# Julian-Wyatt/AnoDDPM

Measured on AMD Instinct MI355X. Metric: reverse-diffusion images/sec @256x256 T=1000 simplex, higher is better.
Workload: dtype f32; 1 GPU; 256x256 simplex(8 oct) T=1000 base128 attn16,8 batch4/GPU (BASELINE config 2); per_gpu_batch=4, global_batch=4, T=1000, parallelism=batch-sharded x1 (no data-path collective), output_finite=True

## Files before the change

anoddpm_amd/csrc/attention.hip:

```cpp
#include "common.h"

namespace {

typedef float f32x4 __attribute__((ext_vector_type(4)));

constexpr int AT_LMAX = 1024;
constexpr int AT_WAVES = 8;
constexpr int AT_NT = AT_WAVES * 64;

template <int CHQ>
__global__ __launch_bounds__(AT_NT) void attention_kernel(const anoddpm_attention_args a)
{
    constexpr int CH = CHQ * 16;
    constexpr int QP = CH + 4;
    constexpr int TPW = CHQ >= AT_WAVES ? CHQ / AT_WAVES : 1;
    __shared__ __attribute__((aligned(16))) float lds[16 * (AT_LMAX + 4) + 16 * QP];
    const int L = a.L, SP = L + 4;
    float *S = lds, *Qs = lds + 16 * (AT_LMAX + 4);
    const int tid = threadIdx.x, lane = tid & 63, wave = tid >> 6;
    const int l16 = lane & 15, kq = lane >> 4;
    const int row0 = blockIdx.x * 16, hd = blockIdx.y, b = blockIdx.z;
    const int C3 = 3 * a.heads * CH;
    const float *__restrict__ qkv = a.qkv + (int64_t)b * L * C3 + hd * 3 * CH;
    const int nkt = L >> 4;

    for (int idx = tid; idx < 16 * (CH / 4); idx += AT_NT) {
        const int r = idx / (CH / 4), c4 = idx - r * (CH / 4);
        *reinterpret_cast<f32x4 *>(Qs + r * QP + c4 * 4) = *reinterpret_cast<const f32x4 *>(qkv + (int64_t)(row0 + r) * C3 + c4 * 4);
    }
    constexpr bool DB = CHQ < 32;
    f32x4 kb[DB ? 2 : 1][CHQ];
    auto load_k = [&](f32x4 (&dst)[CHQ], int jt) {
        const float *kp = qkv + (int64_t)(jt * 16 + l16) * C3 + CH + kq * 4;
#pragma unroll
        for (int g = 0; g < CHQ; ++g) dst[g] = *reinterpret_cast<const f32x4 *>(kp + g * 16);
    };
    constexpr int NACC = CHQ >= 32 ? 4 : 1;
    auto score_tile = [&](const f32x4 (&kk)[CHQ], int jt) {
        f32x4 acc[NACC];
#pragma unroll
        for (int c = 0; c < NACC; ++c) acc[c] = f32x4{0.f, 0.f, 0.f, 0.f};
#pragma unroll
        for (int g = 0; g < CHQ; ++g) {
            const f32x4 qa = *reinterpret_cast<const f32x4 *>(Qs + l16 * QP + g * 16 + kq * 4);
#pragma unroll
            for (int e = 0; e < 4; ++e) acc[g % NACC] = __builtin_amdgcn_mfma_f32_16x16x4f32(qa[e], kk[g][e], acc[g % NACC], 0, 0, 0);
        }
        if constexpr (NACC == 4) acc[0] = (acc[0] + acc[1]) + (acc[2] + acc[3]);
#pragma unroll
        for (int r = 0; r < 4; ++r) S[(kq * 4 + r) * SP + jt * 16 + l16] = acc[0][r] * a.scale;
    };
    if (wave < nkt) load_k(kb[0], wave);
    __syncthreads();
    if constexpr (DB) {
        for (int jt = wave; jt < nkt; jt += 2 * AT_WAVES) {
            if (jt + AT_WAVES < nkt) load_k(kb[1], jt + AT_WAVES);
            score_tile(kb[0], jt);
            if (jt + AT_WAVES < nkt) {
                if (jt + 2 * AT_WAVES < nkt) load_k(kb[0], jt + 2 * AT_WAVES);
                score_tile(kb[1], jt + AT_WAVES);
            }
        }
    } else {
        for (int jt = wave; jt < nkt; jt += AT_WAVES) {
            if (jt != wave) load_k(kb[0], jt);
            score_tile(kb[0], jt);
        }
    }
    const int ct0 = wave * TPW;
    const bool pv_active = ct0 < CHQ;
    float vb[2][TPW][4];
    auto load_v = [&](float (&dst)[TPW][4], int kg) {
        const float *vp = qkv + (int64_t)(kg * 16 + kq * 4) * C3 + 2 * CH + ct0 * 16 + l16;
#pragma unroll
        for (int t = 0; t < TPW; ++t)
#pragma unroll
            for (int e = 0; e < 4; ++e) dst[t][e] = vp[(int64_t)e * C3 + t * 16];
    };
    if (pv_active) load_v(vb[0], 0);
    __syncthreads();

    {
        constexpr int TPR = AT_NT / 16;
        const int r = tid / TPR, sub = tid % TPR;
        float *srow = S + r * SP;
        float m = -INFINITY;
        for (int j = sub; j < L; j += TPR) m = fmaxf(m, srow[j]);
#pragma unroll
        for (int o = TPR / 2; o >= 1; o >>= 1) m = fmaxf(m, __shfl_xor(m, o, TPR));
        float sum = 0.f;
        for (int j = sub; j < L; j += TPR) {
            const float e = __expf(srow[j] - m);
            srow[j] = e;
            sum += e;
        }
#pragma unroll
        for (int o = TPR / 2; o >= 1; o >>= 1) sum += __shfl_xor(sum, o, TPR);
        const float inv = 1.0f / sum;
        float *prow = a.probs ? a.probs + (((int64_t)b * a.heads + hd) * L + row0 + r) * L : nullptr;
        for (int j = sub; j < L; j += TPR) {
            const float p = srow[j] * inv;
            srow[j] = p;
            if (prow) prow[j] = p;
        }
    }
    __syncthreads();

    if (!pv_active) return;
    f32x4 oacc[TPW];
#pragma unroll
    for (int t = 0; t < TPW; ++t) oacc[t] = f32x4{0.f, 0.f, 0.f, 0.f};
    auto pv_group = [&](const float (&vv)[TPW][4], int kg) {
        const f32x4 pa = *reinterpret_cast<const f32x4 *>(S + l16 * SP + kg * 16 + kq * 4);
#pragma unroll
        for (int e = 0; e < 4; ++e)
#pragma unroll
            for (int t = 0; t < TPW; ++t) oacc[t] = __builtin_amdgcn_mfma_f32_16x16x4f32(pa[e], vv[t][e], oacc[t], 0, 0, 0);
    };
    for (int kg = 0; kg < nkt; kg += 2) {
        if (kg + 1 < nkt) load_v(vb[1], kg + 1);
        pv_group(vb[0], kg);
        if (kg + 1 < nkt) {
            if (kg + 2 < nkt) load_v(vb[0], kg + 2);
            pv_group(vb[1], kg + 1);
        }
    }
    float *__restrict__ O = a.out + ((int64_t)b * L + row0 + kq * 4) * (a.heads * CH) + hd * CH + ct0 * 16 + l16;
#pragma unroll
    for (int t = 0; t < TPW; ++t)
#pragma unroll
        for (int r = 0; r < 4; ++r) O[(int64_t)r * (a.heads * CH) + t * 16] = oacc[t][r];
}

}

extern "C" int anoddpm_attention(const anoddpm_attention_args *a, void *stream)
{
    ANODDPM_REQUIRE(a && a->qkv && a->out, "attention: null pointer");
    ANODDPM_REQUIRE(a->B >= 1 && a->heads >= 1 && a->B <= 65535 && a->heads <= 65535, "attention: bad batch / head count");
    ANODDPM_REQUIRE(a->L >= 16 && a->L % 16 == 0 && a->L <= AT_LMAX, "attention: L must be a multiple of 16 in [16, 1024]");
    ANODDPM_REQUIRE(a->ch >= 16 && a->ch <= 512 && (a->ch & (a->ch - 1)) == 0, "attention: head width must be a power of two in [16, 512]");
    ANODDPM_REQUIRE(((uintptr_t)a->qkv & 15) == 0, "attention: qkv must be 16-byte aligned");
    const dim3 grid((unsigned)(a->L / 16), (unsigned)a->heads, (unsigned)a->B);
    hipStream_t s = anoddpm::as_stream(stream);
    switch (a->ch / 16) {
        case 1: hipLaunchKernelGGL((attention_kernel<1>), grid, dim3(AT_NT), 0, s, *a); break;
        case 2: hipLaunchKernelGGL((attention_kernel<2>), grid, dim3(AT_NT), 0, s, *a); break;
        case 4: hipLaunchKernelGGL((attention_kernel<4>), grid, dim3(AT_NT), 0, s, *a); break;
        case 8: hipLaunchKernelGGL((attention_kernel<8>), grid, dim3(AT_NT), 0, s, *a); break;
        case 16: hipLaunchKernelGGL((attention_kernel<16>), grid, dim3(AT_NT), 0, s, *a); break;
        default: hipLaunchKernelGGL((attention_kernel<32>), grid, dim3(AT_NT), 0, s, *a); break;
    }
    return anoddpm::check_launch("attention");
}
```

anoddpm_amd/csrc/winograd.hip:

```cpp
#include "buf_load.h"
#include "common.h"

using anoddpm::buf_load4;
using anoddpm::buf_rsrc;
using anoddpm::f32x4;
using anoddpm::silu_f;

namespace {

typedef float f32x16 __attribute__((ext_vector_type(16)));

constexpr int WKC = 16;

constexpr int DPITCH = 5;

template <bool FAST, int WMW, int WNW, bool PROBE = false, bool VSH = false>
__global__ __launch_bounds__(128 * WMW * WNW, 2) void wino_kernel(const anoddpm_igemm_args a)
{
    unsigned long long tstamp[5];
    if (PROBE) tstamp[0] = __builtin_amdgcn_s_memtime();
    constexpr int NT = 128 * WMW * WNW;
    constexpr int WBN = 32 * WNW;
    constexpr int PROWS = 8 * WMW + 2;
    constexpr int WPATCH = PROWS * 18;
    constexpr int PJ = (WPATCH * 4 + NT - 1) / NT;
    constexpr int SLOTPX = PJ * NT / 4;
    constexpr int DT_F4 = SLOTPX * DPITCH;
    constexpr int EX_FLOATS = (WMW * WNW) * 2 * 8 * 4 * 64;
    constexpr int V_F4 = 16 * 4 * 32;
    constexpr int LDS_FLOATS = VSH ? (2 * DT_F4 + 2 * V_F4) * 4 : EX_FLOATS;
    __shared__ __attribute__((aligned(16))) float lds[LDS_FLOATS];
    static_assert(VSH ? (EX_FLOATS <= LDS_FLOATS && WNW == 4 && WMW == 1) : (2 * DT_F4 * 4 <= EX_FLOATS), "LDS layout");
    static_assert(PJ * NT >= WPATCH * 4 && PJ * NT <= SLOTPX * 4, "staging slots");
    f32x4 *ldsD = reinterpret_cast<f32x4 *>(lds);

    const int tid = threadIdx.x;
    const int lane = tid & 63, wave = tid >> 6;
    const int xh = __builtin_amdgcn_readfirstlane(wave / (WMW * WNW));
    const int wm = (wave / WNW) & (WMW - 1), wn = wave & (WNW - 1);
    const int h = lane >> 5, l31 = lane & 31;

    const int H = a.H, W = a.W;
    const int K = a.c0 + a.c1, N = a.N, K4 = K >> 2;
    const int bx = blockIdx.x % (W >> 4), by = blockIdx.x / (W >> 4);
    const int y0 = by * (8 * WMW), x0 = bx * 16;
    const int n0 = blockIdx.y * WBN;
    const int ksplit = a.ksplit;
    const int ksi = blockIdx.z % ksplit;
    const int b = blockIdx.z / ksplit;
    const int a_mode = a.a_mode;

    const float *A0 = a.a0 + (int64_t)b * a.a0_bs;
    const float *A1 = a.a1 ? a.a1 + (int64_t)b * a.a1_bs : nullptr;
    const float *gsc = a.gn_scale ? a.gn_scale + (int64_t)b * a.gn_ld : nullptr;
    const float *gsh = a.gn_shift ? a.gn_shift + (int64_t)b * a.gn_ld : nullptr;
    const bool affine = (gsc != nullptr);
    const bool act = a.act != 0;
    const int nchunks_all = K / WKC;
    const int cps = (nchunks_all + ksplit - 1) / ksplit;
    const int cbeg = ksi * cps;
    const int nchunks = cbeg + cps < nchunks_all ? cbeg + cps : nchunks_all;

    int spix[PJ];
    const int pq = tid & 3;
#pragma unroll
    for (int j = 0; j < PJ; ++j) {
        const int idx = tid + j * NT;
        const int p = idx >> 2;
        const int py = p / 18, px = p - py * 18;
        const int gy = y0 + py - 1, gx = x0 + px - 1;
        int sp = -1;
        if (p < WPATCH && gy >= 0 && gy < H && gx >= 0 && gx < W)
            sp = (a_mode == 0) ? gy * W + gx : (gy >> 1) * (W >> 1) + (gx >> 1);
        spix[j] = sp;
    }
    f32x4 praw[PJ];
    f32x4 asc = {1.f, 1.f, 1.f, 1.f}, ash = {0.f, 0.f, 0.f, 0.f};
    const __amdgpu_buffer_rsrc_t rA0 = buf_rsrc(A0), rA1 = buf_rsrc(A1 ? A1 : A0);
    const __amdgpu_buffer_rsrc_t rSc = buf_rsrc(gsc ? gsc : A0), rSh = buf_rsrc(gsh ? gsh : A0);
    auto load_patch = [&](int chunk) {
        const int kbase = chunk * WKC;
        const bool first = kbase < a.c0;
// ... 137 lines not shown
                __builtin_amdgcn_sched_barrier(0);
#pragma unroll
                for (int v = 0; v < 4; ++v)
#pragma unroll
                    for (int kk = 0; kk < 4; ++kk)
                        acc[uu * 4 + v] = __builtin_amdgcn_mfma_f32_32x32x2f32(af[set][v][kk], bvr[uu][v][kk], acc[uu * 4 + v], 0, 0, 0);
                __builtin_amdgcn_sched_barrier(0);
                if (g4 < 2) load_b(chunk, 1, uu, uu);
                else        load_b(nxt, 0, uu, uu);
                if (g4 == 0) store_patch(chunk & 1);
                if (g4 == 1) t_write((chunk + 1) & 1);
                if (g4 == 2) load_patch(nxt3);
            }
        }
    } else {
        load_patch(cbeg);
        store_patch(cbeg & 1);
        load_patch(cbeg < last ? cbeg + 1 : last);
        load_b(cbeg, 0, 0, 0);
        load_b(cbeg, 0, 1, 1);
        __syncthreads();
        issue_reads(cbeg & 1, 0, 0, 0);
        issue_reads(cbeg & 1, 0, 0, 1);
        make_av(0);
        if (PROBE) tstamp[1] = __builtin_amdgcn_s_memtime();
        for (int chunk = cbeg; chunk < nchunks; ++chunk) {
            const int nxt = chunk < last ? chunk + 1 : last;
            const int nxt2 = chunk + 2 < nchunks ? chunk + 2 : last;
    #pragma unroll
            for (int g4 = 0; g4 < 4; ++g4) {
                const int uu = g4 & 1;
                if (g4 == 3) __syncthreads();
                const int rbuf = g4 < 3 ? (chunk & 1) : ((chunk + 1) & 1);
                const int rkg = g4 < 3 ? (g4 + 1) >> 1 : 0, ruu = (g4 + 1) & 1;
                issue_reads(rbuf, rkg, ruu, 0);
                __builtin_amdgcn_sched_barrier(0);
    #pragma unroll
                for (int v = 0; v < 2; ++v)
    #pragma unroll
                    for (int kk = 0; kk < 4; ++kk)
                        acc[uu * 4 + v] = __builtin_amdgcn_mfma_f32_32x32x2f32(av[v][kk], bvr[uu][v][kk], acc[uu * 4 + v], 0, 0, 0);
                __builtin_amdgcn_sched_barrier(0);
                issue_reads(rbuf, rkg, ruu, 1);
                __builtin_amdgcn_sched_barrier(0);
    #pragma unroll
                for (int v = 2; v < 4; ++v)
    #pragma unroll
                    for (int kk = 0; kk < 4; ++kk)
                        acc[uu * 4 + v] = __builtin_amdgcn_mfma_f32_32x32x2f32(av[v][kk], bvr[uu][v][kk], acc[uu * 4 + v], 0, 0, 0);
                __builtin_amdgcn_sched_barrier(0);
                if (g4 < 2) load_b(chunk, 1, uu, uu);
                else        load_b(nxt, 0, uu, uu);
                if (g4 == 0) {
                    store_patch((chunk + 1) & 1);
                    load_patch(nxt2);
                }
                make_av(ruu);
            }
        }

    }
    if (PROBE) tstamp[2] = __builtin_amdgcn_s_memtime();
    auto partial = [&](int r, float (&out4)[4]) {
        float tm[2][4];
#pragma unroll
        for (int v = 0; v < 4; ++v) {
            const float m0 = acc[v][r], m1 = acc[4 + v][r];
            if (xh == 0) { tm[0][v] = m0 + m1; tm[1][v] = m1; }
            else         { tm[0][v] = m0;      tm[1][v] = -m0 - m1; }
        }
#pragma unroll
        for (int i = 0; i < 2; ++i) {
            out4[i * 2 + 0] = tm[i][0] + tm[i][1] + tm[i][2];
            out4[i * 2 + 1] = tm[i][1] - tm[i][2] - tm[i][3];
        }
    };
    const int n = n0 + bcol;
    const bool nok = n < N;
    const int nc = nok ? n : 0;
    const bool part = ksplit > 1;
    float *__restrict__ O = part ? a.ws + ((int64_t)ksi * a.B + b) * ((int64_t)H * W) * N : a.out + (int64_t)b * a.o_bs;
    const int o_ld = part ? N : a.out_ld;
    const float alpha = part ? 1.f : a.alpha;
    const float *__restrict__ R = (a.res && !part) ? a.res + (int64_t)b * a.r_bs : nullptr;
    float add = 0.f;
    if (a.bias && !part) add += a.bias[nc];
    if (a.temb && !part) add += a.temb[(int64_t)b * a.temb_ld + nc];
    float cs = 0.f, cq = 0.f;
    float rv[8][4];
#pragma unroll
    for (int rr = 0; rr < 8; ++rr) {
        const int r = xh * 8 + rr;
        const int row = (r & 3) + 8 * (r >> 2) + 4 * h;
        const int tile = wm * 32 + row;
        const int oy = y0 + 2 * (tile >> 3), ox = x0 + 2 * (tile & 7);
#pragma unroll
        for (int e = 0; e < 4; ++e)
            rv[rr][e] = R ? R[((int64_t)(oy + (e >> 1)) * W + ox + (e & 1)) * a.res_ld + nc] : 0.f;
    }
    float *ex = lds;
    const int pair = wave & (WMW * WNW - 1);
    if (xh == 0) {
#pragma unroll
        for (int rr = 0; rr < 8; ++rr) {
            float p4[4];
            partial(8 + rr, p4);
#pragma unroll
            for (int e = 0; e < 4; ++e) ex[(((pair * 2 + 0) * 8 + rr) * 4 + e) * 64 + lane] = p4[e];
        }
    } else {
#pragma unroll
        for (int rr = 0; rr < 8; ++rr) {
            float p4[4];
            partial(rr, p4);
#pragma unroll
            for (int e = 0; e < 4; ++e) ex[(((pair * 2 + 1) * 8 + rr) * 4 + e) * 64 + lane] = p4[e];
        }
    }
    __syncthreads();
    if (PROBE) tstamp[3] = __builtin_amdgcn_s_memtime();

    auto finalize = [&](int rbase) {
#pragma unroll
        for (int rr = 0; rr < 8; ++rr) {
            const int r = rbase + rr;
            const int row = (r & 3) + 8 * (r >> 2) + 4 * h;
            const int tile = wm * 32 + row;
            const int oy = y0 + 2 * (tile >> 3), ox = x0 + 2 * (tile & 7);
            float p4[4];
            partial(r, p4);
#pragma unroll
            for (int e = 0; e < 4; ++e) {
                const float other = ex[(((pair * 2 + (1 - xh)) * 8 + rr) * 4 + e) * 64 + lane];
                const float v = alpha * (p4[e] + other) + add + rv[rr][e];
                if (nok) {
                    O[((int64_t)(oy + (e >> 1)) * W + ox + (e & 1)) * o_ld + nc] = v;
                    cs += v;
                    cq += v * v;
                }
            }
        }
    };
    if (xh == 0) finalize(0); else finalize(8);
    if (a.stats && !part) {
        float *st = a.stats + ((int64_t)b * (gridDim.x * 2 * WMW) + blockIdx.x * (2 * WMW) + wm * 2 + xh) * N * 2;
        const float s2 = cs + __shfl_xor(cs, 32);
        const float q2 = cq + __shfl_xor(cq, 32);
        if (h == 0 && nok) { st[n * 2] = s2; st[n * 2 + 1] = q2; }
    }
    if (PROBE) {
        __builtin_amdgcn_s_waitcnt(0);
        tstamp[4] = __builtin_amdgcn_s_memtime();
        if (tid == 0) {
            unsigned long long *dbg = reinterpret_cast<unsigned long long *>(a.ws) +
                                      (size_t)(blockIdx.x + gridDim.x * (blockIdx.y + gridDim.y * blockIdx.z)) * 8;
            for (int i = 0; i < 5; ++i) dbg[i] = tstamp[i];
        }
    }
}

}

namespace anoddpm {

int launch_winograd(const anoddpm_igemm_args *a, hipStream_t s)
{
    ANODDPM_REQUIRE(a->ks == 3 && a->b_mode == 0 && a->heads == 1, "winograd: needs a 3x3 conv with packed weights");
    ANODDPM_REQUIRE(a->a_mode == 0 || a->a_mode == 1, "winograd: pooled operand loads use the direct kernel");
    ANODDPM_REQUIRE(a->H % 16 == 0 && a->W % 16 == 0, "winograd: H and W must be multiples of 16");
    const int K = a->c0 + a->c1;
    ANODDPM_REQUIRE(K % WKC == 0 && (a->c1 == 0 || a->c0 % WKC == 0), "winograd: channel counts must be multiples of 16");
    const int cps = (K / WKC + a->ksplit - 1) / a->ksplit;
    ANODDPM_REQUIRE((a->ksplit - 1) * cps < K / WKC, "winograd: ksplit leaves a block without channels");
    ANODDPM_REQUIRE(a->ksplit == 1 || !a->stats || a->stats_rows >= 1, "winograd: split-K statistics need stats_rows");
    const int dbg = anoddpm::g_debug[0];
    const int wmw = dbg == 1 ? 2 : 1;
    const bool fast = a->gn_scale && a->act;
#ifdef ANODDPM_ABLATE
    const bool probe = anoddpm::g_debug[1] == 1 && fast && a->ksplit == 1 && a->ws && wmw == 1;
#else
    const bool probe = false;
#endif
    const int wnw = (wmw == 1 && dbg != 2 && !probe && a->N % 128 == 0) ? 4 : 2;
    const int wbn = 32 * wnw;
    dim3 grid((unsigned)wino_tiles(a->H, a->W, wmw), (unsigned)((a->N + wbn - 1) / wbn), (unsigned)(a->B * a->ksplit));
    ANODDPM_REQUIRE(grid.y <= 65535 && (int64_t)a->B * a->ksplit <= 65535, "winograd: grid too large");
    ANODDPM_REQUIRE((int64_t)16 * K * a->N * 4 < ((int64_t)1 << 31), "winograd: transformed weights exceed 32-bit buffer offsets");
    ANODDPM_REQUIRE((int64_t)a->H * a->W * (a->a0_ld > a->a1_ld ? a->a0_ld : a->a1_ld) * 4 < ((int64_t)1 << 31),
                    "winograd: operand slice exceeds 32-bit buffer offsets");
    if (wmw == 2) {
        if (fast) hipLaunchKernelGGL((wino_kernel<true, 2, 2>), grid, dim3(512), 0, s, *a);
        else      hipLaunchKernelGGL((wino_kernel<false, 2, 2>), grid, dim3(512), 0, s, *a);
#ifdef ANODDPM_ABLATE
    } else if (probe) {
        hipLaunchKernelGGL((wino_kernel<true, 1, 2, true>), grid, dim3(256), 0, s, *a);
#endif
    } else if (wnw == 4 && dbg != 3) {
        if (fast) hipLaunchKernelGGL((wino_kernel<true, 1, 4, false, true>), grid, dim3(512), 0, s, *a);
        else      hipLaunchKernelGGL((wino_kernel<false, 1, 4, false, true>), grid, dim3(512), 0, s, *a);
    } else if (wnw == 4) {
        if (fast) hipLaunchKernelGGL((wino_kernel<true, 1, 4>), grid, dim3(512), 0, s, *a);
        else      hipLaunchKernelGGL((wino_kernel<false, 1, 4>), grid, dim3(512), 0, s, *a);
    } else {
        if (fast) hipLaunchKernelGGL((wino_kernel<true, 1, 2>), grid, dim3(256), 0, s, *a);
        else      hipLaunchKernelGGL((wino_kernel<false, 1, 2>), grid, dim3(256), 0, s, *a);
    }
    return check_launch("winograd");
}

}
```

anoddpm_amd/csrc/executor.hip:

```cpp
#include <stdarg.h>
#include <string.h>
#include <vector>
#include "common.h"

namespace anoddpm {

static thread_local char g_err[512] = "";
int g_debug[16] = {0};

void set_error(const char *fmt, ...)
{
    va_list ap;
    va_start(ap, fmt);
    vsnprintf(g_err, sizeof(g_err), fmt, ap);
    va_end(ap);
}

struct ProfState {
    bool on = false;
    std::vector<hipEvent_t> pool;
    std::vector<int> codes;
    std::vector<float> last_ms;
    std::vector<int> last_codes;
    size_t used = 0;
    double ms[ANODDPM_OP_MAX] = {0};
    int64_t launches[ANODDPM_OP_MAX] = {0};
};
static ProfState g_prof;

#define ANODDPM_OPS(X) \
    X(IGEMM,            anoddpm_igemm_args,            anoddpm_igemm) \
    X(GN_STATS,         anoddpm_gn_args,               anoddpm_gn_stats) \
    X(SOFTMAX,          anoddpm_softmax_args,          anoddpm_softmax_rows) \
    X(RESAMPLE,         anoddpm_resample_args,         anoddpm_resample2x) \
    X(LINEAR,           anoddpm_linear_args,           anoddpm_linear_small) \
    X(POSEMB,           anoddpm_posemb_args,           anoddpm_posemb) \
    X(STEM,             anoddpm_stem_args,             anoddpm_conv_stem) \
    X(LAYOUT,           anoddpm_layout_args,           anoddpm_nhwc_to_nchw) \
    X(CHAN_STATS,       anoddpm_chan_stats_args,       anoddpm_chan_stats) \
    X(HEAD,             anoddpm_head_args,             anoddpm_conv_head) \
    X(GN_FINALIZE,      anoddpm_gn_finalize_args,      anoddpm_gn_finalize) \
    X(WGRAD3,           anoddpm_wgrad_args,            anoddpm_conv3x3_wgrad) \
    X(WGRAD1,           anoddpm_wgrad1_args,           anoddpm_wgrad_pointwise) \
    X(GN_BWD,           anoddpm_gn_bwd_args,           anoddpm_gn_silu_backward) \
    X(PACK,             anoddpm_pack_args,             anoddpm_pack_weights) \
    X(SOFTMAX_BWD,      anoddpm_softmax_bwd_args,      anoddpm_softmax_rows_backward) \
    X(TRANSPOSE,        anoddpm_transpose_args,        anoddpm_transpose_square) \
    X(LINEAR_BWD,       anoddpm_linear_bwd_args,       anoddpm_linear_small_backward) \
    X(STEM_BWD,         anoddpm_stem_bwd_args,         anoddpm_conv_stem_backward) \
    X(HEAD_BWD,         anoddpm_head_bwd_args,         anoddpm_conv_head_backward) \
    X(COLSUM_FOLD,      anoddpm_colsum_fold_args,      anoddpm_colsum_fold) \
    X(ATTENTION,        anoddpm_attention_args,        anoddpm_attention) \
    X(PACK_BATCH,       anoddpm_pack_batch_args,       anoddpm_pack_batch) \
    X(DROPOUT,          anoddpm_dropout_args,          anoddpm_dropout) \
    X(LINEAR_BWD_BATCH, anoddpm_linear_bwd_batch_args, anoddpm_linear_small_backward_batch)

static int dispatch(const anoddpm_op &op, void *stream)
{
    switch (op.code) {
#define X(code, args_t, fn) case ANODDPM_OP_##code: return fn(static_cast<const args_t *>(op.args), stream);
        ANODDPM_OPS(X)
#undef X
        default: set_error("run_ops: unknown op code %d", op.code); return ANODDPM_EINVAL;
    }
}

}

using namespace anoddpm;

extern "C" int anoddpm_internal_variant(int32_t key, int32_t value)
{
    if (key < 0 || key >= 16) return ANODDPM_EINVAL;
#ifndef ANODDPM_ABLATE
    if (!(key == 0 || key == 4 || key == 5 || key == 8 || key == 9)) {
        set_error("internal_variant: key %d selects a timing ablation; this library was built without ANODDPM_ABLATE", key);
        return ANODDPM_EINVAL;
    }
#endif
    g_debug[key] = value;
    return ANODDPM_OK;
}

extern "C" int anoddpm_ablate_build(void)
{
#ifdef ANODDPM_ABLATE
    return 1;
#else
    return 0;
#endif
}

extern "C" int anoddpm_abi_version(void) { return ANODDPM_ABI_VERSION; }

extern "C" const char *anoddpm_last_error(void) { return g_err; }

extern "C" int anoddpm_device_count(void)
{
    int n = 0;
    if (hipGetDeviceCount(&n) != hipSuccess) { (void)hipGetLastError(); return 0; }
    return n;
}

extern "C" int anoddpm_run_ops(const anoddpm_op *ops, int32_t n, void *stream)
{
    ANODDPM_REQUIRE(ops || n == 0, "run_ops: null op list");
    for (int i = 0; i < n; ++i) {
        ANODDPM_REQUIRE(ops[i].args, "run_ops: op %d has null args", i);
        hipEvent_t e0 = nullptr, e1 = nullptr;
        const bool prof = g_prof.on && ops[i].code > 0 && ops[i].code < ANODDPM_OP_MAX;
        if (prof) {
            if (g_prof.used + 2 > g_prof.pool.size()) {
                hipEvent_t a, b;
                if (hipEventCreate(&a) != hipSuccess || hipEventCreate(&b) != hipSuccess) {
                    set_error("run_ops: hipEventCreate failed");
                    return ANODDPM_ELAUNCH;
                }
                g_prof.pool.push_back(a);
                g_prof.pool.push_back(b);
            }
            e0 = g_prof.pool[g_prof.used];
            e1 = g_prof.pool[g_prof.used + 1];
            g_prof.used += 2;
            const int icfg = ops[i].code == ANODDPM_OP_IGEMM ? static_cast<const anoddpm_igemm_args *>(ops[i].args)->cfg : 0;
            const bool w43 = ops[i].code == ANODDPM_OP_WGRAD3 && static_cast<const anoddpm_wgrad_args *>(ops[i].args)->algo == 1;
            g_prof.codes.push_back((icfg == 2 || icfg == 6) ? 12 : ((icfg == 3 || icfg == 7) ? 14 : (icfg == 5 ? 13 : (w43 ? 15 : ops[i].code))));
            (void)hipEventRecord(e0, as_stream(stream));
        }
        const int rc = dispatch(ops[i], stream);
        if (prof) (void)hipEventRecord(e1, as_stream(stream));
        if (rc != ANODDPM_OK) {
            char tmp[400];
            strncpy(tmp, g_err, sizeof(tmp) - 1);
            tmp[sizeof(tmp) - 1] = 0;
            set_error("op %d (code %d): %s", i, ops[i].code, tmp);
            return rc;
        }
    }
    return ANODDPM_OK;
}

extern "C" int anoddpm_prof_enable(int32_t enable)
{
    g_prof.on = enable != 0;
    if (enable) {
        g_prof.used = 0;
        g_prof.codes.clear();
        memset(g_prof.ms, 0, sizeof(g_prof.ms));
        memset(g_prof.launches, 0, sizeof(g_prof.launches));
    }
    return ANODDPM_OK;
}

extern "C" int anoddpm_prof_active(void) { return g_prof.on ? 1 : 0; }

extern "C" int anoddpm_prof_collect(double *ms_per_code, int64_t *launches_per_code)
{
    ANODDPM_REQUIRE(ms_per_code && launches_per_code, "prof_collect: null pointer");
// ... 50 lines not shown
```

anoddpm_amd/csrc/smallmap.hip:

```cpp
#include "buf_load.h"
#include "common.h"
#include "gn_stats.h"

using anoddpm::buf_load4;
using anoddpm::buf_rsrc;
using anoddpm::f32x4;
using anoddpm::silu_f;
using anoddpm::uniform;

namespace {

constexpr int SM_NT = 512;

__host__ __device__ constexpr int sm_kch(int ks) { return ks == 3 ? 256 : 512; }
__host__ __device__ constexpr int sm_hpix(int ks, int tm, int w) { return ks == 1 ? tm : (tm / w + 2) * (w + 2); }

template <int KS, int RT, int CT, int LOG2W>
__global__ __launch_bounds__(SM_NT) void smallmap_kernel(const anoddpm_igemm_args a)
{
    constexpr int TM = 16 * RT, TN = 16 * CT, TAPS = KS * KS;
    constexpr int KCH = sm_kch(KS), PITCH = KCH + 4;
    constexpr int CPW = KCH / 8;
    constexpr int SPT = CPW / 16;
    constexpr int SPC = TAPS * SPT;
    constexpr int PD = KS == 3 ? 6 : 4;
    constexpr int W = 1 << LOG2W;
    constexpr int HPIX = sm_hpix(KS, TM, W);
    constexpr int HP = W + 2;
    constexpr int QPP = KCH / 4;
    constexpr int PPI = SM_NT / QPP;
    constexpr int NI = (HPIX + PPI - 1) / PPI;
    constexpr int RP = TN + 4;
    static_assert(SPC % PD == 0, "ring slots must be static");
    extern __shared__ __attribute__((aligned(16))) float lds[];

    const int tid = threadIdx.x, lane = tid & 63;
    const int wave = __builtin_amdgcn_readfirstlane(tid >> 6);
    const int l16 = lane & 15, q = lane >> 4;
    const int K = a.c0 + a.c1, K4 = K >> 2, N = a.N;
    const int P = a.H * a.W;
    const int nchunks = (K + KCH - 1) / KCH;
    const int Kpad = nchunks * KCH;
    const int nbuf = nchunks > 1 ? 2 : 1;
    float *aff_sc = lds, *aff_sh = lds + Kpad;
    float *Abuf = lds + 2 * Kpad;
    float *red = Abuf;

    const int n0 = blockIdx.x * TN;
    const int p0g = blockIdx.y * TM;
    const int b = p0g / P, p0 = p0g - b * P;
    const int y0 = p0 >> LOG2W;
    const float *A0 = a.a0 + (int64_t)b * a.a0_bs;
    const float *A1 = a.a1 ? a.a1 + (int64_t)b * a.a1_bs : A0;

    const __amdgpu_buffer_rsrc_t rW = buf_rsrc(a.bmat);
    const unsigned ulane = ((unsigned)q * (unsigned)N + (unsigned)(n0 + l16)) * 16u;
    const int total_steps = nchunks * SPC;
    auto b_off = [&](int chunk, int s) -> unsigned {
        if (chunk * SPC + s >= total_steps) { chunk = nchunks - 1; s = SPC - 1; }
        const int tap = s / SPT, i = s % SPT;
        int k4 = (chunk * KCH + wave * CPW + 16 * i) >> 2;
        if (k4 + 4 > K4) k4 = 0;
        return ((unsigned)tap * (unsigned)K4 + (unsigned)k4) * (unsigned)N * 16u;
    };
    f32x4 ring[PD][CT];
#pragma unroll
    for (int s = 0; s < PD; ++s) {
        const unsigned o = b_off(0, s);
#pragma unroll
        for (int ct = 0; ct < CT; ++ct) ring[s][ct] = buf_load4(rW, ulane, o + ct * 256u);
    }

    const int kq = tid % QPP;
    int soff[NI];
#pragma unroll
    for (int j = 0; j < NI; ++j) {
        const int hp = tid / QPP + PPI * j;
        int sp = -1;
        if (hp < HPIX) {
            if (KS == 1) sp = p0 + hp;
            else {
                const int hy = hp / HP, hx = hp - hy * HP;
                const int gy = y0 - 1 + hy, gx = hx - 1;
                if (gy >= 0 && gy < a.H && gx >= 0 && gx < W) sp = gy * W + gx;
            }
        }
        soff[j] = sp;
    }
    f32x4 araw[NI];
    unsigned avalid = 0;
    const int ld0 = uniform(a.a0_ld), ld1 = uniform(a.a1_ld);
    auto load_A = [&](int chunk) {
        const int k = chunk * KCH + 4 * kq;
        const bool kv = k < K;
        const bool first = k < a.c0;
        const float *src = first ? A0 + (kv ? k : 0) : A1 + (kv ? k - a.c0 : 0);
        const int ld = first ? ld0 : ld1;
        avalid = 0;
// ... 63 lines not shown
#pragma unroll
            for (int e = 0; e < 4; ++e)
#pragma unroll
                for (int rt = 0; rt < RT; ++rt)
#pragma unroll
                    for (int ct = 0; ct < CT; ++ct)
                        acc[rt][ct] = __builtin_amdgcn_mfma_f32_16x16x4f32(av[cur][rt][e], ring[slot][ct][e], acc[rt][ct], 0, 0, 0);
            const unsigned o = (s + PD < SPC) ? b_off(chunk, s + PD) : b_off(chunk + 1, s + PD - SPC);
#pragma unroll
            for (int ct = 0; ct < CT; ++ct) ring[slot][ct] = buf_load4(rW, ulane, o + ct * 256u);
            __builtin_amdgcn_sched_barrier(0);
        }
        if (more) {
            if (nbuf == 1) __syncthreads();
            store_A(chunk + 1);
        }
        __syncthreads();
    }

    auto red_at = [&](int slot, int rt, int ct, int e) { return red + ((slot * TM + rt * 16 + 4 * q + e) * RP + ct * 16 + l16); };
    if (wave >= 4) {
#pragma unroll
        for (int rt = 0; rt < RT; ++rt)
#pragma unroll
            for (int ct = 0; ct < CT; ++ct)
#pragma unroll
                for (int e = 0; e < 4; ++e) *red_at(wave - 4, rt, ct, e) = acc[rt][ct][e];
    }
    __syncthreads();
    if (wave < 4) {
#pragma unroll
        for (int rt = 0; rt < RT; ++rt)
#pragma unroll
            for (int ct = 0; ct < CT; ++ct)
#pragma unroll
                for (int e = 0; e < 4; ++e) acc[rt][ct][e] += *red_at(wave, rt, ct, e);
    }
    __syncthreads();
    if (wave < 4) {
#pragma unroll
        for (int rt = 0; rt < RT; ++rt)
#pragma unroll
            for (int ct = 0; ct < CT; ++ct)
#pragma unroll
                for (int e = 0; e < 4; ++e) *red_at(wave, rt, ct, e) = acc[rt][ct][e];
    }
    __syncthreads();
    float *O = a.out + (int64_t)b * a.o_bs;
    const float *R = a.res ? a.res + (int64_t)b * a.r_bs : nullptr;
    const float *TE = a.temb ? a.temb + (int64_t)b * a.temb_ld : nullptr;
    constexpr int ITEMS = TM * (TN / 4);
    for (int it = tid; it < ITEMS; it += SM_NT) {
        const int row = it / (TN / 4), c4 = it - row * (TN / 4);
        const float *r0 = red + row * RP + c4 * 4;
        f32x4 v = *reinterpret_cast<const f32x4 *>(r0);
        v += *reinterpret_cast<const f32x4 *>(r0 + TM * RP);
        v += *reinterpret_cast<const f32x4 *>(r0 + 2 * TM * RP);
        v += *reinterpret_cast<const f32x4 *>(r0 + 3 * TM * RP);
        const int n = n0 + c4 * 4;
        v = v * a.alpha;
        if (a.bias) v += *reinterpret_cast<const f32x4 *>(a.bias + n);
        if (TE) v += *reinterpret_cast<const f32x4 *>(TE + n);
        if (R) v += *reinterpret_cast<const f32x4 *>(R + (int64_t)(p0 + row) * a.res_ld + n);
        *reinterpret_cast<f32x4 *>(O + (int64_t)(p0 + row) * a.out_ld + n) = v;
        if (a.stats) *reinterpret_cast<f32x4 *>(red + (4 * TM + row) * RP + c4 * 4) = v;
    }
    if (a.stats) {
        __syncthreads();
        if (tid < TN) {
            const float *col = red + 4 * TM * RP + tid;
            float s = 0.f, qq = 0.f;
#pragma unroll 4
            for (int r = 0; r < TM; ++r) { const float v = col[r * RP]; s += v; qq += v * v; }
            float *st = a.stats + (((int64_t)b * (P / TM) + p0 / TM) * N + n0 + tid) * 2;
            st[0] = s; st[1] = qq;
        }
    }
}

}

namespace anoddpm {

int smallmap_tile(int ks, int H, int W, int K, int c0, int N, int B)
{
    const int P = H * W;
    if (!(ks == 1 || ks == 3) || P > 256 || P < 16 || (W != 4 && W != 8 && W != 16) || H * W != P) return 0;
    if (K % 16 || c0 % 4 || K > 1024 || N % 32 || K < 16) return 0;
    const int M = B * P;
    static const int cand[4][2] = {{2, 6}, {1, 6}, {2, 2}, {1, 2}};
    int best = 0;
    for (int c = 0; c < 4; ++c) {
        const int rt = cand[c][0], ct = cand[c][1];
        const int tm = 16 * rt, tn = 16 * ct;
        if (P % tm || tm % W || N % tn) continue;
        if (ks == 3 && ct == 6) continue;
        const int wgs = (M / tm) * (N / tn);
        if (wgs >= 200) return rt * 16 + ct;
        best = rt * 16 + ct;
    }
    return best;
}

int launch_smallmap(const anoddpm_igemm_args *a, hipStream_t s)
{
    const int K = a->c0 + a->c1;
    ANODDPM_REQUIRE(a->b_mode == 0 && a->heads == 1 && a->a_mode == 0 && a->ksplit == 1, "smallmap: needs packed weights, heads 1, a_mode 0, ksplit 1");
    const int tile = smallmap_tile(a->ks, a->H, a->W, K, a->c0, a->N, a->B);
    ANODDPM_REQUIRE(tile != 0, "smallmap: shape not supported (H*W <= 256, W in {4, 8, 16}, K %% 16 == 0, 16 <= K <= 1024, N %% 32 == 0)");
    ANODDPM_REQUIRE(a->c1 == 0 || a->a1, "smallmap: dual source needs a1");
    ANODDPM_REQUIRE(a->out_ld % 4 == 0 && (!a->res || a->res_ld % 4 == 0) && a->a0_ld % 4 == 0 && (a->c1 == 0 || a->a1_ld % 4 == 0),
                    "smallmap: pixel strides must be multiples of 4 floats");
    ANODDPM_REQUIRE(!a->tail_csum, "smallmap: no split-K tail");
    ANODDPM_REQUIRE(!a->gn_scale || a->gn_shift, "smallmap: gn_scale without gn_shift");
    if (int rc = check_fold_args(a, K, "smallmap")) return rc;
    const int rt = tile >> 4, ct = tile & 15;
    const int TM = 16 * rt, TN = 16 * ct;
    const int P = a->H * a->W;
    const int kch = sm_kch(a->ks);
    const int nchunks = (K + kch - 1) / kch, Kpad = nchunks * kch;
    const int hpix = sm_hpix(a->ks, TM, a->W);
    size_t stage = (size_t)(nchunks > 1 ? 2 : 1) * hpix * (kch + 4) * sizeof(float);
    const size_t fold = (size_t)(2 * Kpad + 128) * sizeof(double);
    const size_t redb = (size_t)5 * TM * (TN + 4) * sizeof(float);
    if (stage < fold) stage = fold;
    if (stage < redb) stage = redb;
    const size_t lds = (size_t)2 * Kpad * sizeof(float) + stage;
    ANODDPM_REQUIRE(lds <= 160 * 1024, "smallmap: LDS budget exceeded");
    dim3 grid((unsigned)(a->N / TN), (unsigned)((int64_t)a->B * smallmap_tiles(P, tile)));
#define SM_LAUNCH(KS_, RT_, CT_, LW_)                                                                                     \
    do {                                                                                                                  \
        static bool attr_done[ANODDPM_MAX_DEV];                                                                           \
        if (int rc_ = allow_big_lds(reinterpret_cast<const void *>(&smallmap_kernel<KS_, RT_, CT_, LW_>), attr_done,      \
                                    "igemm(smallmap)"))                                                                   \
            return rc_;                                                                                                   \
        hipLaunchKernelGGL((smallmap_kernel<KS_, RT_, CT_, LW_>), grid, dim3(SM_NT), lds, s, *a);                         \
        return check_launch("igemm(smallmap)");                                                                           \
    } while (0)
    const int lw = a->W == 4 ? 2 : (a->W == 8 ? 3 : 4);
    if (a->ks == 3) {
        if (rt == 1 && ct == 2) { if (lw == 2) SM_LAUNCH(3, 1, 2, 2); if (lw == 3) SM_LAUNCH(3, 1, 2, 3); SM_LAUNCH(3, 1, 2, 4); }
        if (rt == 2 && ct == 2) { if (lw == 2) SM_LAUNCH(3, 2, 2, 2); if (lw == 3) SM_LAUNCH(3, 2, 2, 3); SM_LAUNCH(3, 2, 2, 4); }
    } else {
        if (rt == 1 && ct == 2) SM_LAUNCH(1, 1, 2, 3);
        if (rt == 1 && ct == 6) SM_LAUNCH(1, 1, 6, 3);
        if (rt == 2 && ct == 2) SM_LAUNCH(1, 2, 2, 3);
        if (rt == 2 && ct == 6) SM_LAUNCH(1, 2, 6, 3);
    }
#undef SM_LAUNCH
    set_error("smallmap: no instantiation for tile %d x %d", TM, TN);
    return ANODDPM_EINVAL;
}

}

extern "C" int anoddpm_smallmap_tile(int32_t ks, int32_t H, int32_t W, int32_t K, int32_t c0, int32_t N, int32_t B)
{
    return anoddpm::smallmap_tile(ks, H, W, K, c0, N, B);
}
```

Before: 0.4525 images/s.

## Deepen attention K/V prefetch pipelines and specialize winograd epilogue residual path

In attention, Q staging now issues all global loads before any LDS stores. For wide heads, the next K tile is prefetched one channel group at a time, interleaved with the score MFMAs. The PV loop now uses a 4- or 8-deep rotating V register prefetch with scheduling barriers, clamping out-of-range loads. In the winograd epilogue, the residual loads are skipped when there is no residual, and the finalize step is specialized at compile time on the row base and on whether a residual exists. The intent is to hide global load latency, at the cost of more registers and possible lower occupancy.

```diff
diff --git a/anoddpm_amd/csrc/attention.hip b/anoddpm_amd/csrc/attention.hip
--- a/anoddpm_amd/csrc/attention.hip
+++ b/anoddpm_amd/csrc/attention.hip
@@ -24,9 +24,20 @@
     const float *__restrict__ qkv = a.qkv + (int64_t)b * L * C3 + hd * 3 * CH;
     const int nkt = L >> 4;
 
-    for (int idx = tid; idx < 16 * (CH / 4); idx += AT_NT) {
-        const int r = idx / (CH / 4), c4 = idx - r * (CH / 4);
-        *reinterpret_cast<f32x4 *>(Qs + r * QP + c4 * 4) = *reinterpret_cast<const f32x4 *>(qkv + (int64_t)(row0 + r) * C3 + c4 * 4);
+    {
+        constexpr int QN = 16 * (CH / 4);
+        constexpr int QPT = (QN + AT_NT - 1) / AT_NT;
+        f32x4 qr[QPT];
+#pragma unroll
+        for (int i = 0; i < QPT; ++i) {
+            const int idx = tid + i * AT_NT, r = idx / (CH / 4), c4 = idx - r * (CH / 4);
+            if (QN % AT_NT == 0 || idx < QN) qr[i] = *reinterpret_cast<const f32x4 *>(qkv + (int64_t)(row0 + r) * C3 + c4 * 4);
+        }
+#pragma unroll
+        for (int i = 0; i < QPT; ++i) {
+            const int idx = tid + i * AT_NT, r = idx / (CH / 4), c4 = idx - r * (CH / 4);
+            if (QN % AT_NT == 0 || idx < QN) *reinterpret_cast<f32x4 *>(Qs + r * QP + c4 * 4) = qr[i];
+        }
     }
     constexpr bool DB = CHQ < 32;
     f32x4 kb[DB ? 2 : 1][CHQ];
@@ -36,7 +47,7 @@
         for (int g = 0; g < CHQ; ++g) dst[g] = *reinterpret_cast<const f32x4 *>(kp + g * 16);
     };
     constexpr int NACC = CHQ >= 32 ? 4 : 1;
-    auto score_tile = [&](const f32x4 (&kk)[CHQ], int jt) {
+    auto score_tile = [&](const f32x4 (&kk)[CHQ], int jt, auto &&after_group) {
         f32x4 acc[NACC];
 #pragma unroll
         for (int c = 0; c < NACC; ++c) acc[c] = f32x4{0.f, 0.f, 0.f, 0.f};
@@ -45,6 +56,7 @@
             const f32x4 qa = *reinterpret_cast<const f32x4 *>(Qs + l16 * QP + g * 16 + kq * 4);
 #pragma unroll
             for (int e = 0; e < 4; ++e) acc[g % NACC] = __builtin_amdgcn_mfma_f32_16x16x4f32(qa[e], kk[g][e], acc[g % NACC], 0, 0, 0);
+            after_group(g);
         }
         if constexpr (NACC == 4) acc[0] = (acc[0] + acc[1]) + (acc[2] + acc[3]);
 #pragma unroll
@@ -55,29 +67,41 @@
     if constexpr (DB) {
         for (int jt = wave; jt < nkt; jt += 2 * AT_WAVES) {
             if (jt + AT_WAVES < nkt) load_k(kb[1], jt + AT_WAVES);
-            score_tile(kb[0], jt);
+            score_tile(kb[0], jt, [](int) {});
             if (jt + AT_WAVES < nkt) {
                 if (jt + 2 * AT_WAVES < nkt) load_k(kb[0], jt + 2 * AT_WAVES);
-                score_tile(kb[1], jt + AT_WAVES);
+                score_tile(kb[1], jt + AT_WAVES, [](int) {});
             }
         }
     } else {
         for (int jt = wave; jt < nkt; jt += AT_WAVES) {
-            if (jt != wave) load_k(kb[0], jt);
-            score_tile(kb[0], jt);
+            if (jt + AT_WAVES < nkt) {
+                const float *kn = qkv + (int64_t)((jt + AT_WAVES) * 16 + l16) * C3 + CH + kq * 4;
+                score_tile(kb[0], jt, [&](int g) {
+                    kb[0][g] = *reinterpret_cast<const f32x4 *>(kn + g * 16);
+                    __builtin_amdgcn_sched_barrier(0);
+                });
+            } else {
+                score_tile(kb[0], jt, [](int) {});
+            }
         }
     }
+    constexpr int VD = TPW >= 4 ? 4 : 8;
     const int ct0 = wave * TPW;
     const bool pv_active = ct0 < CHQ;
-    float vb[2][TPW][4];
+    float vb[VD][TPW][4];
     auto load_v = [&](float (&dst)[TPW][4], int kg) {
+        kg = kg < nkt ? kg : nkt - 1;
         const float *vp = qkv + (int64_t)(kg * 16 + kq * 4) * C3 + 2 * CH + ct0 * 16 + l16;
 #pragma unroll
         for (int t = 0; t < TPW; ++t)
 #pragma unroll
             for (int e = 0; e < 4; ++e) dst[t][e] = vp[(int64_t)e * C3 + t * 16];
     };
-    if (pv_active) load_v(vb[0], 0);
+    if (pv_active) {
+#pragma unroll
+        for (int s = 0; s < VD; ++s) load_v(vb[s], s);
+    }
     __syncthreads();
 
     {
@@ -117,14 +141,18 @@
 #pragma unroll
             for (int t = 0; t < TPW; ++t) oacc[t] = __builtin_amdgcn_mfma_f32_16x16x4f32(pa[e], vv[t][e], oacc[t], 0, 0, 0);
     };
-    for (int kg = 0; kg < nkt; kg += 2) {
-        if (kg + 1 < nkt) load_v(vb[1], kg + 1);
-        pv_group(vb[0], kg);
-        if (kg + 1 < nkt) {
-            if (kg + 2 < nkt) load_v(vb[0], kg + 2);
-            pv_group(vb[1], kg + 1);
+    int kg0 = 0;
+    for (; kg0 + VD <= nkt; kg0 += VD) {
+#pragma unroll
+        for (int s = 0; s < VD; ++s) {
+            pv_group(vb[s], kg0 + s);
+            load_v(vb[s], kg0 + s + VD);
+            __builtin_amdgcn_sched_barrier(0);
         }
     }
+#pragma unroll
+    for (int s = 0; s < VD - 1; ++s)
+        if (kg0 + s < nkt) pv_group(vb[s], kg0 + s);
     float *__restrict__ O = a.out + ((int64_t)b * L + row0 + kq * 4) * (a.heads * CH) + hd * CH + ct0 * 16 + l16;
 #pragma unroll
     for (int t = 0; t < TPW; ++t)
diff --git a/anoddpm_amd/csrc/winograd.hip b/anoddpm_amd/csrc/winograd.hip
--- a/anoddpm_amd/csrc/winograd.hip
+++ b/anoddpm_amd/csrc/winograd.hip
@@ -1,3 +1,5 @@
+#include <type_traits>
+
 #include "buf_load.h"
 #include "common.h"
 
@@ -301,21 +303,23 @@
     float *__restrict__ O = part ? a.ws + ((int64_t)ksi * a.B + b) * ((int64_t)H * W) * N : a.out + (int64_t)b * a.o_bs;
     const int o_ld = part ? N : a.out_ld;
     const float alpha = part ? 1.f : a.alpha;
-    const float *__restrict__ R = (a.res && !part) ? a.res + (int64_t)b * a.r_bs : nullptr;
+    const bool has_res = a.res && !part;
+    const float *__restrict__ R = has_res ? a.res + (int64_t)b * a.r_bs : nullptr;
     float add = 0.f;
     if (a.bias && !part) add += a.bias[nc];
     if (a.temb && !part) add += a.temb[(int64_t)b * a.temb_ld + nc];
     float cs = 0.f, cq = 0.f;
     float rv[8][4];
-#pragma unroll
-    for (int rr = 0; rr < 8; ++rr) {
-        const int r = xh * 8 + rr;
-        const int row = (r & 3) + 8 * (r >> 2) + 4 * h;
-        const int tile = wm * 32 + row;
-        const int oy = y0 + 2 * (tile >> 3), ox = x0 + 2 * (tile & 7);
-#pragma unroll
-        for (int e = 0; e < 4; ++e)
-            rv[rr][e] = R ? R[((int64_t)(oy + (e >> 1)) * W + ox + (e & 1)) * a.res_ld + nc] : 0.f;
+    if (has_res) {
+#pragma unroll
+        for (int rr = 0; rr < 8; ++rr) {
+            const int r = xh * 8 + rr;
+            const int row = (r & 3) + 8 * (r >> 2) + 4 * h;
+            const int tile = wm * 32 + row;
+            const int oy = y0 + 2 * (tile >> 3), ox = x0 + 2 * (tile & 7);
+#pragma unroll
+            for (int e = 0; e < 4; ++e) rv[rr][e] = R[((int64_t)(oy + (e >> 1)) * W + ox + (e & 1)) * a.res_ld + nc];
+        }
     }
     float *ex = lds;
     const int pair = wave & (WMW * WNW - 1);
@@ -339,7 +343,10 @@
     __syncthreads();
     if (PROBE) tstamp[3] = __builtin_amdgcn_s_memtime();
 
-    auto finalize = [&](int rbase) {
+    auto finalize = [&](auto rbase_c, auto res_c) {
+        constexpr int rbase = decltype(rbase_c)::value;
+        constexpr bool RES = decltype(res_c)::value;
+        if (!nok) return;
 #pragma unroll
         for (int rr = 0; rr < 8; ++rr) {
             const int r = rbase + rr;
@@ -351,16 +358,20 @@
 #pragma unroll
             for (int e = 0; e < 4; ++e) {
                 const float other = ex[(((pair * 2 + (1 - xh)) * 8 + rr) * 4 + e) * 64 + lane];
-                const float v = alpha * (p4[e] + other) + add + rv[rr][e];
-                if (nok) {
-                    O[((int64_t)(oy + (e >> 1)) * W + ox + (e & 1)) * o_ld + nc] = v;
-                    cs += v;
-                    cq += v * v;
-                }
+                const float v = alpha * (p4[e] + other) + add + (RES ? rv[rr][e] : 0.f);
+                O[((int64_t)(oy + (e >> 1)) * W + ox + (e & 1)) * o_ld + nc] = v;
+                cs += v;
+                cq += v * v;
             }
         }
     };
-    if (xh == 0) finalize(0); else finalize(8);
+    using rb0 = std::integral_constant<int, 0>;
+    using rb8 = std::integral_constant<int, 8>;
+    if (has_res) {
+        if (xh == 0) finalize(rb0{}, std::true_type{}); else finalize(rb8{}, std::true_type{});
+    } else {
+        if (xh == 0) finalize(rb0{}, std::false_type{}); else finalize(rb8{}, std::false_type{});
+    }
     if (a.stats && !part) {
         float *st = a.stats + ((int64_t)b * (gridDim.x * 2 * WMW) + blockIdx.x * (2 * WMW) + wm * 2 + xh) * N * 2;
         const float s2 = cs + __shfl_xor(cs, 32);
```

Result: no change. 0.4537 images/s (median of 6 runs) (+0.3%).

## Deepen V prefetch pipeline, register-cache softmax rows, add forced smallmap tile option

Applied to the files above, without the earlier changes.

The attention PV loop now prefetches V tiles several stages deep (7 or 3 register buffers), with sched barriers to keep loads ahead of the MFMAs. The Q staging issues all global loads before any LDS stores. Softmax keeps each thread's score slice in registers across the max, exp and normalise passes, so LDS is read once instead of three times. Smallmap gains a debug-forced tile selection (key 10), a new 32x16 ks=3 instantiation and a shared LDS-size helper. The deeper V buffers add register pressure and may reduce occupancy.

```diff
diff --git a/anoddpm_amd/csrc/attention.hip b/anoddpm_amd/csrc/attention.hip
--- a/anoddpm_amd/csrc/attention.hip
+++ b/anoddpm_amd/csrc/attention.hip
@@ -24,9 +24,19 @@
     const float *__restrict__ qkv = a.qkv + (int64_t)b * L * C3 + hd * 3 * CH;
     const int nkt = L >> 4;
 
-    for (int idx = tid; idx < 16 * (CH / 4); idx += AT_NT) {
-        const int r = idx / (CH / 4), c4 = idx - r * (CH / 4);
-        *reinterpret_cast<f32x4 *>(Qs + r * QP + c4 * 4) = *reinterpret_cast<const f32x4 *>(qkv + (int64_t)(row0 + r) * C3 + c4 * 4);
+    {
+        constexpr int QITEMS = 16 * (CH / 4), QN = (QITEMS + AT_NT - 1) / AT_NT;
+        f32x4 qraw[QN];
+#pragma unroll
+        for (int j = 0; j < QN; ++j) {
+            const int idx = tid + j * AT_NT, r = idx / (CH / 4), c4 = idx - r * (CH / 4);
+            if (QITEMS % AT_NT == 0 || idx < QITEMS) qraw[j] = *reinterpret_cast<const f32x4 *>(qkv + (int64_t)(row0 + r) * C3 + c4 * 4);
+        }
+#pragma unroll
+        for (int j = 0; j < QN; ++j) {
+            const int idx = tid + j * AT_NT, r = idx / (CH / 4), c4 = idx - r * (CH / 4);
+            if (QITEMS % AT_NT == 0 || idx < QITEMS) *reinterpret_cast<f32x4 *>(Qs + r * QP + c4 * 4) = qraw[j];
+        }
     }
     constexpr bool DB = CHQ < 32;
     f32x4 kb[DB ? 2 : 1][CHQ];
@@ -69,39 +79,74 @@
     }
     const int ct0 = wave * TPW;
     const bool pv_active = ct0 < CHQ;
-    float vb[2][TPW][4];
+    constexpr int VD = TPW <= 2 ? 7 : 3;
+    float vb[VD][TPW][4];
     auto load_v = [&](float (&dst)[TPW][4], int kg) {
+        kg = min(kg, nkt - 1);
         const float *vp = qkv + (int64_t)(kg * 16 + kq * 4) * C3 + 2 * CH + ct0 * 16 + l16;
 #pragma unroll
         for (int t = 0; t < TPW; ++t)
 #pragma unroll
             for (int e = 0; e < 4; ++e) dst[t][e] = vp[(int64_t)e * C3 + t * 16];
     };
-    if (pv_active) load_v(vb[0], 0);
+    if (pv_active) {
+#pragma unroll
+        for (int s = 0; s < VD; ++s) {
+            load_v(vb[s], s);
+            __builtin_amdgcn_sched_barrier(0);
+        }
+    }
     __syncthreads();
 
     {
         constexpr int TPR = AT_NT / 16;
         const int r = tid / TPR, sub = tid % TPR;
         float *srow = S + r * SP;
+        constexpr int SCH = 8, NCH = AT_LMAX / (TPR * SCH);
+        float sv[NCH][SCH];
         float m = -INFINITY;
-        for (int j = sub; j < L; j += TPR) m = fmaxf(m, srow[j]);
+#pragma unroll
+        for (int c = 0; c < NCH; ++c) {
+            if (c * TPR * SCH >= L) break;
+#pragma unroll
+            for (int i = 0; i < SCH; ++i) {
+                const int j = sub + TPR * (c * SCH + i);
+                sv[c][i] = j < L ? srow[j] : -INFINITY;
+            }
+#pragma unroll
+            for (int i = 0; i < SCH; ++i) m = fmaxf(m, sv[c][i]);
+        }
 #pragma unroll
         for (int o = TPR / 2; o >= 1; o >>= 1) m = fmaxf(m, __shfl_xor(m, o, TPR));
         float sum = 0.f;
-        for (int j = sub; j < L; j += TPR) {
-            const float e = __expf(srow[j] - m);
-            srow[j] = e;
-            sum += e;
+#pragma unroll
+        for (int c = 0; c < NCH; ++c) {
+            if (c * TPR * SCH >= L) break;
+#pragma unroll
+            for (int i = 0; i < SCH; ++i) {
+                const int j = sub + TPR * (c * SCH + i);
+                if (j < L) {
+                    sv[c][i] = __expf(sv[c][i] - m);
+                    sum += sv[c][i];
+                }
+            }
         }
 #pragma unroll
         for (int o = TPR / 2; o >= 1; o >>= 1) sum += __shfl_xor(sum, o, TPR);
         const float inv = 1.0f / sum;
         float *prow = a.probs ? a.probs + (((int64_t)b * a.heads + hd) * L + row0 + r) * L : nullptr;
-        for (int j = sub; j < L; j += TPR) {
-            const float p = srow[j] * inv;
-            srow[j] = p;
-            if (prow) prow[j] = p;
+#pragma unroll
+        for (int c = 0; c < NCH; ++c) {
+            if (c * TPR * SCH >= L) break;
+#pragma unroll
+            for (int i = 0; i < SCH; ++i) {
+                const int j = sub + TPR * (c * SCH + i);
+                if (j < L) {
+                    const float p = sv[c][i] * inv;
+                    srow[j] = p;
+                    if (prow) prow[j] = p;
+                }
+            }
         }
     }
     __syncthreads();
@@ -117,13 +162,19 @@
 #pragma unroll
             for (int t = 0; t < TPW; ++t) oacc[t] = __builtin_amdgcn_mfma_f32_16x16x4f32(pa[e], vv[t][e], oacc[t], 0, 0, 0);
     };
-    for (int kg = 0; kg < nkt; kg += 2) {
-        if (kg + 1 < nkt) load_v(vb[1], kg + 1);
-        pv_group(vb[0], kg);
-        if (kg + 1 < nkt) {
-            if (kg + 2 < nkt) load_v(vb[0], kg + 2);
-            pv_group(vb[1], kg + 1);
-        }
+    int kg0 = 0;
+    for (; kg0 + VD < nkt; kg0 += VD) {
+#pragma unroll
+        for (int s = 0; s < VD; ++s) {
+            pv_group(vb[s], kg0 + s);
+            load_v(vb[s], kg0 + s + VD);
+            __builtin_amdgcn_sched_barrier(0);
+        }
+    }
+#pragma unroll
+    for (int s = 0; s < VD; ++s) {
+        if (kg0 + s >= nkt) break;
+        pv_group(vb[s], kg0 + s);
     }
     float *__restrict__ O = a.out + ((int64_t)b * L + row0 + kq * 4) * (a.heads * CH) + hd * CH + ct0 * 16 + l16;
 #pragma unroll
diff --git a/anoddpm_amd/csrc/executor.hip b/anoddpm_amd/csrc/executor.hip
--- a/anoddpm_amd/csrc/executor.hip
+++ b/anoddpm_amd/csrc/executor.hip
@@ -73,7 +73,7 @@
 {
     if (key < 0 || key >= 16) return ANODDPM_EINVAL;
 #ifndef ANODDPM_ABLATE
-    if (!(key == 0 || key == 4 || key == 5 || key == 8 || key == 9)) {
+    if (!(key == 0 || key == 4 || key == 5 || key == 8 || key == 9 || key == 10)) {
         set_error("internal_variant: key %d selects a timing ablation; this library was built without ANODDPM_ABLATE", key);
         return ANODDPM_EINVAL;
     }
diff --git a/anoddpm_amd/csrc/smallmap.hip b/anoddpm_amd/csrc/smallmap.hip
--- a/anoddpm_amd/csrc/smallmap.hip
+++ b/anoddpm_amd/csrc/smallmap.hip
@@ -14,6 +14,19 @@
 
 __host__ __device__ constexpr int sm_kch(int ks) { return ks == 3 ? 256 : 512; }
 __host__ __device__ constexpr int sm_hpix(int ks, int tm, int w) { return ks == 1 ? tm : (tm / w + 2) * (w + 2); }
+
+constexpr size_t SM_LDS_MAX = 160 * 1024;
+size_t sm_lds_bytes(int ks, int tm, int tn, int W, int K)
+{
+    const int kch = sm_kch(ks);
+    const int nchunks = (K + kch - 1) / kch, Kpad = nchunks * kch;
+    size_t stage = (size_t)(nchunks > 1 ? 2 : 1) * sm_hpix(ks, tm, W) * (kch + 4) * sizeof(float);
+    const size_t fold = (size_t)(2 * Kpad + 128) * sizeof(double);
+    const size_t redb = (size_t)5 * tm * (tn + 4) * sizeof(float);
+    if (stage < fold) stage = fold;
+    if (stage < redb) stage = redb;
+    return (size_t)2 * Kpad * sizeof(float) + stage;
+}
 
 template <int KS, int RT, int CT, int LOG2W>
 __global__ __launch_bounds__(SM_NT) void smallmap_kernel(const anoddpm_igemm_args a)
@@ -243,19 +256,30 @@
 
 namespace anoddpm {
 
+static bool sm_tile_fits(int ks, int H, int W, int K, int N, int rt, int ct)
+{
+    const int tm = 16 * rt, tn = 16 * ct;
+    if (!(rt == 1 || rt == 2) || !(ct == 1 || ct == 2 || ct == 6) || (rt == 1 && ct == 1)) return false;
+    if ((H * W) % tm || tm % W || N % tn) return false;
+    if (ks == 3 ? (ct == 6) : (ct == 1)) return false;
+    return sm_lds_bytes(ks, tm, tn, W, K) <= SM_LDS_MAX;
+}
+
 int smallmap_tile(int ks, int H, int W, int K, int c0, int N, int B)
 {
     const int P = H * W;
     if (!(ks == 1 || ks == 3) || P > 256 || P < 16 || (W != 4 && W != 8 && W != 16) || H * W != P) return 0;
-    if (K % 16 || c0 % 4 || K > 1024 || N % 32 || K < 16) return 0;
+    if (K % 16 || c0 % 4 || K > 1024 || K < 16) return 0;
+    const int forced = g_debug[10];
+    if (forced > 0 && N % 16 == 0 && sm_tile_fits(ks, H, W, K, N, forced >> 4, forced & 15)) return forced;
+    if (N % 32) return 0;
     const int M = B * P;
     static const int cand[4][2] = {{2, 6}, {1, 6}, {2, 2}, {1, 2}};
     int best = 0;
     for (int c = 0; c < 4; ++c) {
         const int rt = cand[c][0], ct = cand[c][1];
         const int tm = 16 * rt, tn = 16 * ct;
-        if (P % tm || tm % W || N % tn) continue;
-        if (ks == 3 && ct == 6) continue;
+        if (!sm_tile_fits(ks, H, W, K, N, rt, ct)) continue;
         const int wgs = (M / tm) * (N / tn);
         if (wgs >= 200) return rt * 16 + ct;
         best = rt * 16 + ct;
@@ -278,16 +302,8 @@
     const int rt = tile >> 4, ct = tile & 15;
     const int TM = 16 * rt, TN = 16 * ct;
     const int P = a->H * a->W;
-    const int kch = sm_kch(a->ks);
-    const int nchunks = (K + kch - 1) / kch, Kpad = nchunks * kch;
-    const int hpix = sm_hpix(a->ks, TM, a->W);
-    size_t stage = (size_t)(nchunks > 1 ? 2 : 1) * hpix * (kch + 4) * sizeof(float);
-    const size_t fold = (size_t)(2 * Kpad + 128) * sizeof(double);
-    const size_t redb = (size_t)5 * TM * (TN + 4) * sizeof(float);
-    if (stage < fold) stage = fold;
-    if (stage < redb) stage = redb;
-    const size_t lds = (size_t)2 * Kpad * sizeof(float) + stage;
-    ANODDPM_REQUIRE(lds <= 160 * 1024, "smallmap: LDS budget exceeded");
+    const size_t lds = sm_lds_bytes(a->ks, TM, TN, a->W, K);
+    ANODDPM_REQUIRE(lds <= SM_LDS_MAX, "smallmap: LDS budget exceeded");
     dim3 grid((unsigned)(a->N / TN), (unsigned)((int64_t)a->B * smallmap_tiles(P, tile)));
 #define SM_LAUNCH(KS_, RT_, CT_, LW_)                                                                                     \
     do {                                                                                                                  \
@@ -301,6 +317,7 @@
     const int lw = a->W == 4 ? 2 : (a->W == 8 ? 3 : 4);
     if (a->ks == 3) {
         if (rt == 1 && ct == 2) { if (lw == 2) SM_LAUNCH(3, 1, 2, 2); if (lw == 3) SM_LAUNCH(3, 1, 2, 3); SM_LAUNCH(3, 1, 2, 4); }
+        if (rt == 2 && ct == 1) { if (lw == 2) SM_LAUNCH(3, 2, 1, 2); if (lw == 3) SM_LAUNCH(3, 2, 1, 3); SM_LAUNCH(3, 2, 1, 4); }
         if (rt == 2 && ct == 2) { if (lw == 2) SM_LAUNCH(3, 2, 2, 2); if (lw == 3) SM_LAUNCH(3, 2, 2, 3); SM_LAUNCH(3, 2, 2, 4); }
     } else {
         if (rt == 1 && ct == 2) SM_LAUNCH(1, 1, 2, 3);
```

Result: no change. 0.4480 images/s before, 0.4489 images/s after (median of 6 runs) (+0.2%).
